# roljon/Steered-Mixture-of-Experts

Hardware: AMD Instinct MI355X
Metric: Mpixel-iters/s (SMoE fit: forward + analytic backward + TF1 Adam), 16x16 blocks / 4 kernels (higher is better)
Workload: dtype f32

## Files before the change

### steered_mixture_of_experts_amd/csrc/smoe_block.hip.h

```cpp
#ifndef SMOE_BLOCK_HIP_H
#define SMOE_BLOCK_HIP_H

#include <hip/hip_runtime.h>
#include <stdint.h>

#include <type_traits>

#include "smoe_device.h"
#include "smoe_ssim.hip.h"
#include "smoe_fq.hip.h"

namespace smoe {


__device__ __forceinline__ float fast_rcp(float x) { return __builtin_amdgcn_rcpf(x); }

__device__ __forceinline__ uint32_t hw_wave_slot() {
    return __builtin_amdgcn_s_getreg(4 | (0 << 6) | ((4 - 1) << 11));
}
__device__ __forceinline__ void rotate_priority(int it, uint32_t slot) {
    const uint32_t pr = ((uint32_t)it + slot) % 3u;
    if (pr == 0u) __builtin_amdgcn_s_setprio(0);
    else if (pr == 1u) __builtin_amdgcn_s_setprio(1);
    else __builtin_amdgcn_s_setprio(2);
// ... 51 lines not shown
        case 2: return s.A_diagonal;
        case 3: return s.A_corr;
        case 4: return s.gamma_e;
        default: return s.nu_e;
    }
}

#ifndef SMOE_REGRED
#define SMOE_REGRED 0
#endif
#ifndef SMOE_W2_SLOTS
#define SMOE_W2_SLOTS 96
#endif
#ifndef SMOE_W2_G16
#define SMOE_W2_G16 1
#endif
#ifndef SMOE_W2_G32
#define SMOE_W2_G32 1
#endif
#ifndef SMOE_W2_SLOTS_MAX
#define SMOE_W2_SLOTS_MAX 150
#endif
#ifndef SMOE_NT_STORES
#define SMOE_NT_STORES 1
#endif
#ifndef SMOE_SGPR_CONSTS
#define SMOE_SGPR_CONSTS 1
#endif
#ifndef SMOE_PHASE_CLOCKS
#define SMOE_PHASE_CLOCKS 0
#endif
#if SMOE_PHASE_CLOCKS
#define SMOE_CLK(i) do { const unsigned long long _t = __builtin_amdgcn_s_memtime(); clk[i] += (float)(_t - clk_last); clk_last = __builtin_amdgcn_s_memtime(); } while (0)
#else
#define SMOE_CLK(i) do { } while (0)
#endif
#ifndef SMOE_DEBUG
#define SMOE_DEBUG 0
#endif
#if SMOE_DEBUG
#define SMOE_LDS_CHECK(end_floats, code)                                                   \
    do {                                                                                   \
        if ((long)(end_floats) > (long)a.lds_floats) {                                     \
            if (threadIdx.x == 0 && a.dbg != nullptr) atomicOr(a.dbg, (uint32_t)(code));   \
            return;                                                                        \
        }                                                                                  \
    } while (0)
#else
#define SMOE_LDS_CHECK(end_floats, code) do { } while (0)
#endif
#define SMOE_SQ 0.84932180028801904272f
#define SMOE_INV_SQ 1.17740022503374817543f

template <int D, int C, int K>
struct BlockRegs {
    using Lt = Layout<D, C, K>;
    float P[Lt::LP_STRIDE];
    float As[K][Lt::TRI];
    float cz[K][D];
    float coef[K];
    float hz[K][D];
    float he[K][C];
    float hq[K];

    __device__ __forceinline__ float pi(int k) const { return P[k * Lt::PK + Lt::O_PI]; }
    __device__ __forceinline__ float mu(int k, int l) const { return P[k * Lt::PK + Lt::O_MU + l]; }
    __device__ __forceinline__ float A(int k, int l, int m) const { return P[k * Lt::PK + Lt::O_A + tri_index(l, m)]; }
    __device__ __forceinline__ float nu(int k, int c) const { return P[k * Lt::PK + Lt::O_NU + c]; }
    __device__ __forceinline__ float ga(int k, int l, int c) const { return P[k * Lt::PK + Lt::O_GA + l * C + c]; }
    __device__ __forceinline__ bool flag(int k) const { return P[Lt::LP_ACT + k] != 0.0f; }
    __device__ __forceinline__ bool frozen() const { return P[Lt::LP_FROZEN] != 0.0f; }
    __device__ __forceinline__ bool act(int k) const { return flag(k) && (pi(k) > 0.0f); }

    __device__ __forceinline__ void load(const float* __restrict__ lds_block) {
        const float4* src = reinterpret_cast<const float4*>(lds_block);
#pragma unroll
        for (int i = 0; i < Lt::LP_STRIDE / 4; ++i) {
            const float4 q = src[i];
            P[4 * i + 0] = q.x; P[4 * i + 1] = q.y; P[4 * i + 2] = q.z; P[4 * i + 3] = q.w;
        }
    }

    template <bool IC = false>
    __device__ __forceinline__ void derive(const KernelConsts& kc) {
#pragma unroll
        for (int k = 0; k < K; ++k) {
            float det = 1.0f;
#pragma unroll
            for (int l = 0; l < D; ++l) det *= A(k, l, l);
            const float nq = kc.use_det ? det * kc.inv_n_dis : 1.0f;
            coef[k] = act(k) ? nq * pi(k) : 0.0f;
#pragma unroll
            for (int l = 0; l < D; ++l)
#pragma unroll
                for (int m = 0; m <= l; ++m)
                    As[k][tri_index(l, m)] = (IC ? ((l == m) ? SMOE_SQ * SMOE_SQ : 2.0f * SMOE_SQ * SMOE_SQ) : SMOE_SQ) * A(k, l, m);
#pragma unroll
            for (int m = 0; m < D; ++m) {
                float c = 0.0f;
                if (!IC) {
#pragma unroll
                    for (int l = m; l < D; ++l) c = fmaf(mu(k, l), As[k][tri_index(l, m)], c);
                }
                cz[k][m] = c;
            }
            if (!kc.train_gammas) {
#pragma unroll
                for (int i = 0; i < D * C; ++i) P[k * Lt::PK + Lt::O_GA + i] = 0.0f;
            }
            if (kc.only_y_gamma) {
#pragma unroll
                for (int l = 0; l < D; ++l)
#pragma unroll
                    for (int c = 1; c < C; ++c) P[k * Lt::PK + Lt::O_GA + l * C + c] = 0.0f;
            }
        }
    }
};

template <int D, int C, int K>
struct BlockRanges {
    FqRange ad, ac, mu, nu, ga;
    float lo[5], hi[5];
    __device__ __forceinline__ void compute(const float* P, const bool (&keep)[K], const KernelConsts& kc) {
        using Lt = Layout<D, C, K>;
        constexpr float INF = __builtin_huge_valf();
#pragma unroll
        for (int t = 0; t < 5; ++t) { lo[t] = INF; hi[t] = -INF; }
        bool any = false;
#pragma unroll
        for (int k = 0; k < K; ++k) {
            if (!keep[k]) continue;
            any = true;
            const float* p = P + k * Lt::PK;
#pragma unroll
            for (int l = 0; l < D; ++l) {
                lo[2] = fminf(lo[2], p[Lt::O_MU + l]); hi[2] = fmaxf(hi[2], p[Lt::O_MU + l]);
#pragma unroll
                for (int m = 0; m <= l; ++m) {
                    const float a = p[Lt::O_A + tri_index(l, m)];
                    const int t = (l == m) ? 0 : 1;
                    lo[t] = fminf(lo[t], a); hi[t] = fmaxf(hi[t], a);
                }
            }
#pragma unroll
            for (int c = 0; c < C; ++c) { lo[3] = fminf(lo[3], p[Lt::O_NU + c]); hi[3] = fmaxf(hi[3], p[Lt::O_NU + c]); }
#pragma unroll
            for (int i = 0; i < D * C; ++i) { lo[4] = fminf(lo[4], p[Lt::O_GA + i]); hi[4] = fmaxf(hi[4], p[Lt::O_GA + i]); }
        }
// ... 241 lines not shown
#pragma unroll
            for (int l = m; l < D - HL; ++l)
                a[Lt::O_A + tri_index(l, m)] = fmaf(x[l], uz, a[Lt::O_A + tri_index(l, m)]);
        }
        }
#pragma unroll
        for (int c = 0; c < C; ++c) {
            a[Lt::O_NU + c] = fmaf(o.wt[k], Gc[c], a[Lt::O_NU + c]);
#pragma unroll
            for (int l = 0; l < D - HL; ++l)
                a[Lt::O_GA + l * C + c] = fmaf(o.wt[k], Gx[l][c], a[Lt::O_GA + l * C + c]);
        }
    }
}

template <int D, int C, int K, int HL, bool IC = false>
__device__ __forceinline__ void complete_const(const BlockRegs<D, C, K>& R, const float (&xc)[D], float* __restrict__ acc) {
    using Lt = Layout<D, C, K>;
#pragma unroll
    for (int k = 0; k < K; ++k) {
        float* a = acc + k * Lt::PK;
        if (!IC) {
#pragma unroll
            for (int m = D - HL; m < D; ++m) a[Lt::O_MU + m] = R.hz[k][m] * a[Lt::O_PI];
        }
#pragma unroll
        for (int l = D - HL; l < D; ++l) {
            if (IC) {
                const float rl = xc[l] - R.mu(k, l);
#pragma unroll
                for (int m = 0; m <= l; ++m)
                    a[Lt::O_A + tri_index(l, m)] = (m < D - HL) ? rl * a[Lt::O_MU + m] : rl * ((xc[m] - R.mu(k, m)) * a[Lt::O_PI]);
                a[Lt::O_MU + l] = rl * a[Lt::O_PI];
            } else {
#pragma unroll
            for (int m = 0; m <= l; ++m) a[Lt::O_A + tri_index(l, m)] = xc[l] * a[Lt::O_MU + m];
            }
#pragma unroll
            for (int c = 0; c < C; ++c) a[Lt::O_GA + l * C + c] = xc[l] * a[Lt::O_NU + c];
        }
    }
}

template <int D, int C, int K>
__device__ __forceinline__ void tie_diagonal(float* __restrict__ a) {
    using Lt = Layout<D, C, K>;
    float tr = 0.0f;
#pragma unroll
    for (int l = 0; l < D; ++l) tr += a[Lt::O_A + tri_index(l, l)];
#pragma unroll
    for (int l = 0; l < D; ++l) a[Lt::O_A + tri_index(l, l)] = tr;
}

template <int D, int C, int K, bool IC = false>
__device__ __forceinline__ void finish_partials(const BlockRegs<D, C, K>& R, const KernelConsts& kc,
                                                float* __restrict__ acc) {
    using Lt = Layout<D, C, K>;
#pragma unroll
    for (int k = 0; k < K; ++k) {
        float* a = acc + k * Lt::PK;
        const bool act = R.act(k);
        const float su = a[Lt::O_PI];
        if (IC) {
            float sur[D];
#pragma unroll
            for (int l = 0; l < D; ++l) sur[l] = a[Lt::O_MU + l];
#pragma unroll
            for (int l = 0; l < D; ++l) {
                float gm = 0.0f;
#pragma unroll
                for (int m = 0; m < D; ++m) gm = fmaf((l >= m) ? R.A(k, l, m) : R.A(k, m, l), sur[m], gm);
                a[Lt::O_MU + l] = gm;
#pragma unroll
                for (int m = 0; m <= l; ++m) {
                    float v = (l == m) ? -0.5f * a[Lt::O_A + tri_index(l, m)] : -a[Lt::O_A + tri_index(l, m)];
                    if (l == m && kc.use_det) v = fmaf(su, act ? fast_rcp(R.A(k, l, l)) : 0.0f, v);
                    a[Lt::O_A + tri_index(l, m)] = v;
                }
            }
            a[Lt::O_PI] = su * (act ? fast_rcp(R.pi(k)) : 0.0f);
            if (kc.radial) tie_diagonal<D, C, K>(a);
            continue;
        }
        float suz[D];
#pragma unroll
        for (int m = 0; m < D; ++m) suz[m] = a[Lt::O_MU + m] * SMOE_INV_SQ;
#pragma unroll
        for (int l = 0; l < D; ++l) {
            float gm = 0.0f;
#pragma unroll
            for (int m = 0; m <= l; ++m) gm = fmaf(R.A(k, l, m), suz[m], gm);
            a[Lt::O_MU + l] = gm;
        }
#pragma unroll
        for (int l = 0; l < D; ++l) {
#pragma unroll
            for (int m = 0; m <= l; ++m) {
                float v = fmaf(R.mu(k, l), suz[m], -(a[Lt::O_A + tri_index(l, m)] * SMOE_INV_SQ));
                if (l == m && kc.use_det) v = fmaf(su, act ? fast_rcp(R.A(k, l, l)) : 0.0f, v);
                a[Lt::O_A + tri_index(l, m)] = v;
            }
        }
        a[Lt::O_PI] = su * (act ? fast_rcp(R.pi(k)) : 0.0f);
        if (kc.radial) tie_diagonal<D, C, K>(a);
    }
}

struct SlotDesc {
    float c_self, pub_scale;
    uint32_t T1, T2, T3, TR, P1, P2, P3, PR, FLAG, PIV;
};

template <int D, int C, int K, bool IC>
__device__ __forceinline__ SlotDesc build_slot_desc(int j, uint32_t tot_base, uint32_t img_base, uint32_t par_base,
                                                    bool patch_pis, bool use_det) {
    using Lt = Layout<D, C, K>;
    const uint32_t ZERO = par_base + 4u * Lt::LP_ZERO, ONE = par_base + 4u * Lt::LP_ONE;
    const int k = j / Lt::PK, o = j - k * Lt::PK;
    const uint32_t Tk = tot_base + 4u * (uint32_t)(k * Lt::PK), Pk = img_base + 4u * (uint32_t)(k * Lt::PK);
    SlotDesc d;
    d.c_self = 1.0f; d.pub_scale = 1.0f;
    d.T1 = d.T2 = d.T3 = d.TR = ZERO;
    d.P1 = d.P2 = d.P3 = ZERO;
    d.PR = ONE;
    d.FLAG = img_base + 4u * (uint32_t)(Lt::LP_ACT + k);
    d.PIV = patch_pis ? par_base + 4u * (uint32_t)(Lt::LP_QPI + k) : Pk + 4u * Lt::O_PI;
    if (o == Lt::O_PI) {
        d.c_self = 0.0f; d.TR = Tk + 4u * Lt::O_PI; d.PR = d.PIV;
    } else if (o < Lt::O_A) {
        const int l = o - Lt::O_MU;
        d.c_self = 0.0f;
        d.pub_scale = IC ? 1.0f : SMOE_INV_SQ;
        int n = 0;
#pragma unroll
        for (int m = 0; m < D; ++m) {
            if (IC || m <= l) {
                const int hi = (l > m) ? l : m, lo = (l > m) ? m : l;
                const uint32_t P = Pk + 4u * (uint32_t)(Lt::O_A + hi * (hi + 1) / 2 + lo), T = Tk + 4u * (uint32_t)(Lt::O_MU + m);
                if (n == 0) { d.P1 = P; d.T1 = T; } else if (n == 1) { d.P2 = P; d.T2 = T; } else { d.P3 = P; d.T3 = T; }
                ++n;
            }
        }
    } else if (o < Lt::O_NU) {
        const int t = o - Lt::O_A;
        const int l = (t >= 3) ? 2 : ((t >= 1) ? 1 : 0);
        const int m = t - l * (l + 1) / 2;
        if (IC) {
            d.c_self = (l == m) ? -0.5f : -1.0f;
        } else {
            d.c_self = -SMOE_INV_SQ;
            d.P1 = Pk + 4u * (uint32_t)(Lt::O_MU + l);
            d.T1 = Tk + 4u * (uint32_t)(Lt::O_MU + m);
        }
        if (l == m && use_det) { d.TR = Tk + 4u * Lt::O_PI; d.PR = Pk + 4u * (uint32_t)(Lt::O_A + l * (l + 1) / 2 + l); }
    }
    return d;
// ... 21 lines not shown
        return (t == 0) ? 1 : ((t == 1) ? D : ((t == 2 || t == 3) ? D * D : ((t == 4) ? D * C : C)));
    }
    __host__ __device__ static constexpr int before(int t) {
        int n = 0;
        for (int u = 0; u < t; ++u) n += elems(u);
        return n;
    }
    static constexpr int PER_KERNEL = before(6);
};

template <int D, int C, int K, int G, int WAVES>
struct Tile {
    using Lt = Layout<D, C, K>;
    static constexpr int BPW = 64 / G;
    static constexpr int NB = WAVES * BPW;
    static constexpr int U = (G == 64) ? ((Lt::NSLOT >= 90) ? 16 : 32) : G;
    static constexpr int UL = G / U;
    static constexpr int RPR = 64 / UL / (64 / G);
    static constexpr int NROUND = (Lt::NSLOT + RPR - 1) / RPR;
    static constexpr int CH = RPR;
    static constexpr int RPP = CH / RPR;
    static constexpr int ROW = 64 + 4;
    static constexpr int NCHUNK = (Lt::NSLOT + CH - 1) / CH;
    static constexpr bool REGRED = (G == 64) && (SMOE_REGRED != 0);
    static constexpr int RM = (Lt::NSLOT + 3) / 4;
    static constexpr int SPL = REGRED ? (RM + 15) / 16 : (NROUND + UL - 1) / UL;
    __host__ __device__ static constexpr int slot_of(int sub, int s) {
        if (REGRED) {
            const int i = (sub % 16) + 16 * s;
            return (i < RM) ? (sub / 16) * RM + i : Lt::NSLOT;
        }
        return (UL * s + (sub % UL)) * RPR + sub / UL;
    }
    static constexpr int THREADS = WAVES * 64;
    static constexpr int FWD_PXR = 16;
    static_assert(NB * K * ParamTile<D, C, K>::PER_KERNEL <= WAVES * CH * ROW, "the parameter tile of a workgroup is staged in the reduction scratch");
    static constexpr int MV_STRIDE = round_up(2 * Lt::NPAR, 4);
    static constexpr int TGT_PAD = 0;
    __host__ __device__ static constexpr int tgt_stride(int N) { return C * N + TGT_PAD; }
    __host__ __device__ static constexpr int lw_stride(int N) { return N + TGT_PAD; }
    
    __host__ __device__ static int off_coords() { return 0; }
    __host__ __device__ static int off_par(int N, int CR) { return round_up(CR * N, 4); }
    __host__ __device__ static int off_mv(int N, int CR) { return off_par(N, CR) + NB * Lt::LP_STRIDE; }
    static constexpr bool OWNER_POST = (G >= 64);
    static constexpr int DESC_DW = 12;
    static constexpr int DESC_STRIDE = OWNER_POST ? Lt::NPAR * DESC_DW : 0;
    static constexpr int TOT_STRIDE = round_up(Lt::NSLOT, 4);
    static_assert(!OWNER_POST || BPW * TOT_STRIDE <= CH * ROW, "the published totals must fit into the reduction scratch");
    __host__ __device__ static bool wants_owner_post(int N) { return OWNER_POST && N <= 8 * G; }
    __host__ __device__ static int off_scratch(int N, int CR) { return off_mv(N, CR) + NB * MV_STRIDE; }
    __host__ __device__ static int off_tgt(int N, int CR) { return off_scratch(N, CR) + WAVES * CH * ROW; }
    __host__ __device__ static int off_lw(int N, int CR) { return off_tgt(N, CR) + NB * tgt_stride(N); }
    __host__ __device__ static size_t bytes(int N, bool has_lw, int CR = D, bool hq = false) {
        return sizeof(float) * (size_t)off_ssim(N, has_lw, CR, hq);
    }
    static constexpr int QI_RNG = 40;
    static constexpr int QI_OUT = 12;
    static constexpr int QI_STRIDE = round_up(Lt::LP_STRIDE + QI_RNG + QI_OUT, 4);
    __host__ __device__ static int off_qimg(int N, bool has_lw, int CR) { return round_up(off_lw(N, CR) + (has_lw ? NB * lw_stride(N) : 0), 4); }
    __host__ __device__ static int off_ssim(int N, bool has_lw, int CR, bool hq = false) { return off_qimg(N, has_lw, CR) + (hq ? NB * QI_STRIDE : 0); }
    __host__ __device__ static int ssim_tabs(int bh, int bw, int bt = 0) { return (G == 16) ? 0 : round_up(11 * (bh + bw + bt), 4); }
    __host__ __device__ static int ssim_wave(int N) { return (G == 16) ? BPW * C * N : round_up(C * N + ((D == 3) ? 10 : 8) * N, 4); }
    __host__ __device__ static size_t bytes_ssim(int N, bool has_lw, int CR, int bh, int bw, bool hq = false, int bt = 0) {
        return sizeof(float) * (size_t)(off_ssim(N, has_lw, CR, hq) + ssim_tabs(bh, bw, bt) + WAVES * ssim_wave(N));
    }
};

template <int D, int C, int K, int G, int WAVES, int CR = D>
__device__ __forceinline__ void stage_inputs(const float* __restrict__ coords, const float* __restrict__ target,
                                             const float* __restrict__ loss_w, int B, int N, int blk0,
                                             float* __restrict__ lds, bool planes = true) {
    using T = Tile<D, C, K, G, WAVES>;
    static_assert(T::TGT_PAD == 0, "the staged planes of a workgroup are one contiguous run");
    float* s_coords = lds + T::off_coords();
    float* s_tgt = lds + T::off_tgt(N, CR);
    float* s_lw = lds + T::off_lw(N, CR);
    auto copy_planes = [&](const float* __restrict__ src, float* __restrict__ dst, int per) {
        const size_t g0 = (size_t)blk0 * per;
        const size_t gend = (size_t)B * per;
        if ((per & 3) == 0) {
            const float4* __restrict__ src4 = reinterpret_cast<const float4*>(src);
            const size_t last4 = (gend >> 2) - 1;
            for (int i = threadIdx.x; i < T::NB * (per >> 2); i += T::THREADS)
                reinterpret_cast<float4*>(dst)[i] = src4[min((g0 >> 2) + (size_t)i, last4)];
        } else {
            for (int i = threadIdx.x; i < T::NB * per; i += T::THREADS) dst[i] = src[min(g0 + (size_t)i, gend - 1)];
        }
    };
    for (int i = threadIdx.x; i < CR * N; i += T::THREADS) s_coords[i] = coords[i];
    if (!planes) return;
    copy_planes(target, s_tgt, C * N);
    if (loss_w != nullptr) copy_planes(loss_w, s_lw, N);
}

template <int D, int C, int K, int NB, int THREADS>
struct TileIO {
    using PT = ParamTile<D, C, K>;
    static constexpr int TOTAL = NB * K * PT::PER_KERNEL;
    static constexpr int MAXE = (TOTAL + THREADS - 1) / THREADS;
    __device__ static __forceinline__ void locate(int i, int& t, int& local) {
        t = 0; local = i;
#pragma unroll
        for (int u = 1; u < 6; ++u)
            if (i >= NB * K * PT::before(u)) { t = u; local = i - NB * K * PT::before(u); }
    }
    __device__ static __forceinline__ void fetch(const smoe_params& s, int blk0, int B, float (&v)[MAXE]) {
#pragma unroll
        for (int e = 0; e < MAXE; ++e) {
// ... 340 lines not shown
            for (int l = 0; l < D; ++l) x[l] = (l < D - HL) ? s_coords[l * N + n] : 0.0f;
#pragma unroll
            for (int c = 0; c < C; ++c) t[c] = s_tgt[c * N + n];
            const float lw = HAS_LW ? s_lw[n] : 1.0f;
            PixelOut<D, C, K> o;
            pixel<D, C, K, true, HL, false, IC, false, RAWL>(R, kc, x, t, lw, acc, o, nullptr, nullptr, !(HAS_LW && sample) || lw != 0.0f, lraw);
        }
    }
    if constexpr (RAWL) {
#pragma unroll
        for (int c = 0; c < C; ++c) acc[Layout<D, C, K>::S_LOSS] = fmaf(kc.cw[c], lraw[c], acc[Layout<D, C, K>::S_LOSS]);
    }
    const int lane = threadIdx.x & 63;
#pragma unroll
    for (int k = 0; k < K; ++k) acc[Layout<D, C, K>::S_CNT + k] += ((flags[k] >> lane) & 1ull) ? 1.0f : 0.0f;
}

template <int D, int C, int K, int G, int HL, bool SSIM, bool QUANT>
constexpr int fit_min_waves() {
    return ((G == 64 || (G == 16 && SMOE_W2_G16) || (G == 32 && SMOE_W2_G32)) && HL >= 1 && !SSIM && !QUANT && Layout<D, C, K>::NSLOT >= ((G == 64) ? SMOE_W2_SLOTS : 90)
            && Layout<D, C, K>::NSLOT <= SMOE_W2_SLOTS_MAX) ? 2 : 1;
}

template <int D, int C, int K, int G, int WAVES, int HL, bool SSIM = false, bool QUANT = false, bool IC = false, bool PAIR = false>
__global__ void __launch_bounds__(WAVES * 64) __attribute__((amdgpu_waves_per_eu(fit_min_waves<D, C, K, G, HL, SSIM, QUANT>()))) fit_kernel(FitArgs a) {
    using Lt = Layout<D, C, K>;
    using T = Tile<D, C, K, G, WAVES>;
    static_assert(!PAIR || (G == 64 && WAVES == 2 && !SSIM && !QUANT), "PAIR: one block on the two wavefronts of a workgroup");
    extern __shared__ __attribute__((aligned(16))) float lds[];
    const int N = a.N;
    const int B = a.B;
    const int wave = threadIdx.x >> 6;
    const int lane = threadIdx.x & 63;
    const int grp = lane / G;
    const int sub = lane - grp * G;
    const int blk0 = blockIdx.x * (PAIR ? 1 : T::NB);
    const int lb = PAIR ? 0 : wave * T::BPW + grp;
    const bool helper = PAIR && wave != 0;
    const int b_raw = blk0 + lb;
    const bool valid_b = b_raw < B;
    const int b = valid_b ? b_raw : B - 1;

    constexpr int CR = D - HL;
    float* s_coords = lds + T::off_coords();
    float* s_par = lds + T::off_par(N, CR) + lb * Lt::LP_STRIDE;
    float* s_mv = lds + T::off_mv(N, CR) + lb * T::MV_STRIDE;
    float* s_scratch = lds + T::off_scratch(N, CR) + wave * (T::CH * T::ROW);
    const bool owner_post = T::OWNER_POST && a.desc_off > 0;
    float* s_desc = lds + a.desc_off + lb * T::DESC_STRIDE;
    float* s_tot = s_scratch + grp * T::TOT_STRIDE;
    const float* s_tgt = lds + T::off_tgt(N, CR) + lb * T::tgt_stride(N);
    const float* s_lw = lds + T::off_lw(N, CR) + lb * T::lw_stride(N);
    const bool has_lw = a.loss_w != nullptr;

    SMOE_LDS_CHECK(T::off_ssim(N, has_lw, CR, QUANT) + (SSIM ? T::ssim_tabs(a.bh, a.bw, (D == 3) ? a.bt : 0) + WAVES * T::ssim_wave(N) : 0), 1u);
    if (owner_post) SMOE_LDS_CHECK(a.desc_off + T::NB * T::DESC_STRIDE, 2u);
    stage_inputs<D, C, K, G, WAVES, CR>(a.coords, a.target, a.loss_w, B, N, blk0, lds);
    float* s_q = lds + T::off_qimg(N, has_lw, CR) + lb * T::QI_STRIDE;
    float* s_rng = s_q + Lt::LP_STRIDE;
    float* s_out = s_rng + T::QI_RNG;
    float* s_ssim = lds + T::off_ssim(N, has_lw, CR, QUANT);
    const int bh = a.bh, bw = a.bw, bt = (D == 3) ? a.bt : 0;
    const float* s_Tr = s_ssim;
    const float* s_Tc = s_ssim + bh * 11;
    const float* s_Tt = s_Tc + bw * 11;
    float* s_X = s_ssim + T::ssim_tabs(bh, bw, bt) + wave * T::ssim_wave(N) + ((G == 16) ? grp * (C * N) : 0);
    float* s_Wa = s_X + C * N;
    float* s_Wb = s_Wa + 5 * N;
    float wj[11];
    if (SSIM) {
        if (G == 16) {
#pragma unroll
            for (int q = 0; q < 11; ++q) {
                wj[q] = a.ssim_T[11 * 16 + sub * 11 + q];
            }
        } else {
            for (int i = threadIdx.x; i < 11 * (bh + bw + bt); i += T::THREADS) s_ssim[i] = a.ssim_T[i];
        }
    }
    float xc[D];
#pragma unroll
    for (int l = 0; l < D; ++l) xc[l] = a.coords[l * N + min(sub, N - 1)];

    constexpr int QS = QUANT ? T::SPL : 1;
    float lr[T::SPL], reg[T::SPL], qlo[QS], qhi[QS], qsc[QS], qiv[QS];
    float goff[QS];
    int meta[T::SPL], qt[QS];
#pragma unroll
    for (int s = 0; s < QS; ++s) {
        qlo[s] = -__builtin_huge_valf(); qhi[s] = __builtin_huge_valf();
        qsc[s] = qiv[s] = 0.0f;
        qt[s] = -1;
        goff[s] = 0.0f;
    }
#pragma unroll
    for (int s = 0; s < T::SPL; ++s) {
        const int j = T::slot_of(sub, s);
        lr[s] = reg[s] = 0.0f;
        meta[s] = -1;
        if (j < Lt::NPAR) {
            int tensor, kern; long off;
            decode_slot<D, C, K>(j, b, tensor, off, kern);
            s_par[j] = pick(a.p, tensor)[off];
            s_mv[2 * j] = pick(a.m, tensor)[off];
            s_mv[2 * j + 1] = pick(a.v, tensor)[off];
            float r = (tensor == 0) ? a.lr_pis : ((tensor == 2 || tensor == 3) ? a.lr_steer : a.lr_expert);
            if (tensor == 0 && !a.train_pis) r = 0.0f;
            if (tensor == 1 && !a.train_musx) r = 0.0f;
// ... 66 lines not shown
                        o[0] = r.nmin; o[1] = r.nmax; o[2] = r.scale; o[3] = r.inv;
                        o[4] = r.back; o[5] = r.zero ? 1.0f : 0.0f; o[6] = lo; o[7] = hi;
                    }
                }
                wave_lds_sync();
            }
        }
        if constexpr (!QUANT) {
#pragma unroll
            for (int s = 0; s < T::SPL; ++s) {
                const int j = T::slot_of(sub, s);
                if (meta[s] >= 0 && (meta[s] & 15) == 0) {
                    const float x = s_par[j];
                    const float cl = fminf(fmaxf(x, a.kc.q_nmin[3]), a.kc.q_nmax[3]);
                    s_par[Lt::LP_QPI + (meta[s] >> 4)] = floorf((cl - a.kc.q_nmin[3]) * a.kc.q_inv[3] + 0.5f) * a.kc.q_scale[3] + a.kc.q_nmin[3];
                }
            }
            wave_lds_sync();
            return;
        }
        if constexpr (QUANT) {
#pragma unroll
        for (int s = 0; s < T::SPL; ++s) {
            const int j = T::slot_of(sub, s);
            if (j < Lt::NPAR) {
                const float x = s_par[j] - goff[s];
                float q = x;
                if (qsc[s] != 0.0f) {
                    const float cl = fminf(fmaxf(x, qlo[s]), qhi[s]);
                    q = floorf((cl - qlo[s]) * qiv[s] + 0.5f) * qsc[s] + qlo[s];
                }
                {
                    if (qt[s] >= 0) {
                        const float* o = s_rng + qt[s] * 8;
                        FqRange r;
                        r.nmin = o[0]; r.nmax = o[1]; r.scale = o[2]; r.inv = o[3]; r.back = o[4]; r.zero = o[5] != 0.0f;
                        r.shift = (qt[s] == 0 && a.kc.radial) ? 0.0f : r.back;
                        q = fq_val(x, r);
                    }
                }
                s_q[j] = q + goff[s];
            } else if (j >= Lt::S_CNT && j < Lt::S_CNT + K) {
                s_q[Lt::LP_ACT + (j - Lt::S_CNT)] = s_par[Lt::LP_ACT + (j - Lt::S_CNT)];
            } else if (j == Lt::S_LOSS) {
                s_q[Lt::LP_FROZEN] = s_par[Lt::LP_FROZEN];
            }
        }
        }
        wave_lds_sync();
    };
    if (has_quant) refresh_quantised_image();
    const float* s_img = (QUANT && has_quant) ? s_q : s_par;
    const bool patch_pis = !QUANT && (a.kc.qpis != 0);
    if (owner_post && !helper) {
        const uint32_t tot_off = (uint32_t)((s_tot - lds) * sizeof(float));
        const uint32_t img_off = (uint32_t)((s_img - lds) * sizeof(float));
        const uint32_t par_off = (uint32_t)((s_par - lds) * sizeof(float));
#pragma unroll
        for (int s = 0; s < T::SPL; ++s) {
            const int j = T::slot_of(sub, s);
            if (j < Lt::NPAR) {
                const SlotDesc d = build_slot_desc<D, C, K, IC>(j, tot_off, img_off, par_off, patch_pis, a.kc.use_det != 0);
                float4* o = reinterpret_cast<float4*>(s_desc + j * T::DESC_DW);
                o[0] = make_float4(d.c_self, d.pub_scale, __uint_as_float(d.T1), __uint_as_float(d.T2));
                o[1] = make_float4(__uint_as_float(d.T3), __uint_as_float(d.TR), __uint_as_float(d.P1), __uint_as_float(d.P2));
                o[2] = make_float4(__uint_as_float(d.P3), __uint_as_float(d.PR), __uint_as_float(d.FLAG), __uint_as_float(d.PIV));
            } else if (j == Lt::S_LOSS) {
                s_par[Lt::LP_ZERO] = 0.0f;
                s_par[Lt::LP_ONE] = 1.0f;
            }
        }
        wave_lds_sync();
    }

    float b1p = a.b1p, b2p = a.b2p;
    const KernelConsts kc = a.kc;
    const float beta1 = a.beta1, beta2 = a.beta2, adam_eps = a.eps, clip = a.clip;
    const float reg_pi = a.reg_pi, reg_u = a.reg_u;

#if SMOE_PHASE_CLOCKS
    float clk[8] = {0.0f, 0.0f, 0.0f, 0.0f, 0.0f, 0.0f, 0.0f, 0.0f};
    unsigned long long clk_last = __builtin_amdgcn_s_memtime();
#endif
    const bool phase_prio = !PAIR && (G < 64 || N >= 8 * G);
    for (int it = 0; it < a.n_iters; ++it) {
        if (a.prio_rotate) rotate_priority(it, hw_wave_slot());
        else if (phase_prio) __builtin_amdgcn_s_setprio(0);
        float acc[Lt::NSLOT];
#pragma unroll
        for (int j = 0; j < Lt::NSLOT; ++j) acc[j] = 0.0f;
        bool frozen;
        float reg_loss = 0.0f;
        {
            BlockRegs<D, C, K> R;
            R.load(s_img);
            if (patch_pis) {
#pragma unroll
                for (int k = 0; k < K; ++k) R.P[k * Lt::PK + Lt::O_PI] = R.P[Lt::LP_QPI + k];
            }
            R.template derive<IC>(kc);
            frozen = R.frozen();
            if (has_reg) {
                const float rp = kc.kcount_norm ? kc.pis_l1_raw / count_pis<D, C, K>(R.P) : reg_pi;
#pragma unroll
                for (int k = 0; k < K; ++k) {
                    if (R.act(k)) {
                        reg_loss += rp * R.pi(k);
#pragma unroll
                        for (int l = 0; l < D; ++l) reg_loss += reg_u * R.A(k, l, l);
                    }
                }
            }
            if (HL > 0) hoist_const<D, C, K, HL, IC>(R, xc);
#if SMOE_SGPR_CONSTS
            if constexpr (G == 64 && !SSIM && !QUANT && !IC && HL >= 1 && K * C >= 24) {
                auto uni = [](float x) { return __int_as_float(__builtin_amdgcn_readfirstlane(__float_as_int(x))); };
#pragma unroll
                for (int k = 0; k < K; ++k) {
                    R.coef[k] = uni(R.coef[k]);
#pragma unroll
                    for (int l = 0; l < D - HL; ++l) {
#pragma unroll
                        for (int m = 0; m <= l; ++m) R.As[k][tri_index(l, m)] = uni(R.As[k][tri_index(l, m)]);
#pragma unroll
                        for (int c = 0; c < C; ++c) R.P[k * Lt::PK + Lt::O_GA + l * C + c] = uni(R.P[k * Lt::PK + Lt::O_GA + l * C + c]);
                    }
                }
            }
#endif
            SMOE_CLK(0);
            if constexpr (SSIM) {
                const int pxl = (N + G - 1) / G;
                const int full = (G == 16) ? N / G : 0;
                auto recon_step = [&](int n) {
                    float x[D], t[C], scratch_acc[Lt::NSLOT];
#pragma unroll
                    for (int l = 0; l < D; ++l) x[l] = (l < D - HL) ? s_coords[l * N + n] : 0.0f;
#pragma unroll
                    for (int c = 0; c < C; ++c) t[c] = s_tgt[c * N + n];
#pragma unroll
                    for (int j = 0; j < Lt::NSLOT; ++j) scratch_acc[j] = 0.0f;
                    PixelOut<D, C, K> o;
                    pixel<D, C, K, false, HL, false, IC>(R, kc, x, t, 1.0f, scratch_acc, o);
#pragma unroll
                    for (int c = 0; c < C; ++c) s_X[c * N + n] = o.q[c];
                };
                for (int i = 0; i < full; ++i) recon_step(i * G + sub);
                for (int i = full; i < pxl; ++i)
                    if (i * G + sub < N) recon_step(i * G + sub);
                wave_lds_sync();
                if constexpr (G == 16) acc[Lt::S_LOSS] = ssim_block16<C, true>(s_X, s_tgt, sub, wj, kc.sw);
                else if constexpr (D == 3) acc[Lt::S_LOSS] = ssim_block3<C, true>(s_X, s_tgt, s_Wa, s_Wb, s_Tr, s_Tc, s_Tt, kc.sw, bh, bw, bt, N, lane);
                else acc[Lt::S_LOSS] = ssim_block<C, true>(s_X, s_tgt, s_Wa, s_Wb, s_Tr, s_Tc, kc.sw, bh, bw, N, lane);
                unsigned long long flags[K];
#pragma unroll
                for (int k = 0; k < K; ++k) flags[k] = 0ull;
                auto grad_step = [&](int n, auto voted) {
                    float x[D], t[C], gq[C];
#pragma unroll
                    for (int l = 0; l < D; ++l) x[l] = (l < D - HL) ? s_coords[l * N + n] : 0.0f;
#pragma unroll
                    for (int c = 0; c < C; ++c) { t[c] = s_tgt[c * N + n]; gq[c] = s_X[c * N + n]; }
                    PixelOut<D, C, K> o;
                    pixel<D, C, K, true, HL, true, IC, decltype(voted)::value>(R, kc, x, t, 1.0f, acc, o, gq, flags);
                };
                for (int i = 0; i < full; ++i) grad_step(i * G + sub, std::true_type{});
                for (int i = full; i < pxl; ++i)
                    if (i * G + sub < N) grad_step(i * G + sub, std::false_type{});
#pragma unroll
                for (int k = 0; k < K; ++k) acc[Lt::S_CNT + k] += ((flags[k] >> lane) & 1ull) ? 1.0f : 0.0f;
            } else {
                const int gl = PAIR ? 2 * G : G, sl = PAIR ? wave * G + sub : sub;
                if (has_lw) pixel_loop_train<D, C, K, true, HL, IC>(R, kc, s_coords, s_tgt, s_lw, N, gl, sl, acc, a.lw_is_sample != 0);
                else pixel_loop_train<D, C, K, false, HL, IC>(R, kc, s_coords, s_tgt, s_lw, N, gl, sl, acc);
            }
            if (HL > 0) complete_const<D, C, K, HL, IC>(R, xc, acc);
            SMOE_CLK(1);
        }
        if (phase_prio) __builtin_amdgcn_s_setprio(3);
        if (!owner_post) {
            BlockRegs<D, C, K> R2;
            R2.load(s_img);
            if (patch_pis) {
#pragma unroll
                for (int k = 0; k < K; ++k) R2.P[k * Lt::PK + Lt::O_PI] = R2.P[Lt::LP_QPI + k];
            }
            finish_partials<D, C, K, IC>(R2, kc, acc);
        }

        SMOE_CLK(2);
        float total[T::SPL];
        reduce_slots<D, C, K, G, WAVES, 0>(acc, s_scratch, lane, total);
        SMOE_CLK(3);

        if constexpr (PAIR) {
            float* s_x = lds + T::off_scratch(N, CR) + (T::CH * T::ROW);
            if (helper) {
                wave_lds_sync();
#pragma unroll
                for (int s = 0; s < T::SPL; ++s) {
                    const int j = T::slot_of(sub, s);
                    if (j < Lt::NSLOT) s_x[j] = total[s];
                }
            }
            __syncthreads();
            if (helper) {
                __syncthreads();
                b1p *= beta1;
                b2p *= beta2;
                SMOE_CLK(4);
                continue;
            }
#pragma unroll
            for (int s = 0; s < T::SPL; ++s) {
                const int j = T::slot_of(sub, s);
                if (j < Lt::NSLOT) total[s] += s_x[j];
            }
        }

        SMOE_CLK(4);
        if (owner_post) {
            SlotDesc dsc[T::SPL];
#pragma unroll
            for (int s = 0; s < T::SPL; ++s) {
                int j = T::slot_of(sub, s);
                asm volatile("" : "+v"(j));
                const int jc = (j < Lt::NPAR) ? j : 0;
                const float4* q = reinterpret_cast<const float4*>(s_desc + jc * T::DESC_DW);
                const float4 q0 = q[0], q1 = q[1], q2 = q[2];
                dsc[s].c_self = q0.x; dsc[s].pub_scale = q0.y; dsc[s].T1 = __float_as_uint(q0.z); dsc[s].T2 = __float_as_uint(q0.w);
                dsc[s].T3 = __float_as_uint(q1.x); dsc[s].TR = __float_as_uint(q1.y); dsc[s].P1 = __float_as_uint(q1.z); dsc[s].P2 = __float_as_uint(q1.w);
                dsc[s].P3 = __float_as_uint(q2.x); dsc[s].PR = __float_as_uint(q2.y); dsc[s].FLAG = __float_as_uint(q2.z); dsc[s].PIV = __float_as_uint(q2.w);
                if (j < Lt::NPAR) s_tot[j] = total[s] * dsc[s].pub_scale;
            }
            wave_lds_sync();
#pragma unroll
            for (int s = 0; s < T::SPL; ++s) {
                const int j = T::slot_of(sub, s);
                if (j < Lt::NPAR) total[s] = eval_slot_desc(lds, dsc[s], total[s]);
            }
// ... 87 lines not shown
                        float g = (bel[s] || abv[s]) ? 0.0f : gq[s];
                        g += tlo[s] ? pick5(rs, 0, qt[s]) / fmaxf(pick5(cn, 0, qt[s]), 1.0f) : 0.0f;
                        g += thi[s] ? pick5(rs, 5, qt[s]) / fmaxf(pick5(cn, 5, qt[s]), 1.0f) : 0.0f;
                        gq[s] = g;
                    }
                }
            }
        }
        float newp[T::SPL], newm[T::SPL], newv[T::SPL], pvs[T::SPL], mvs[T::SPL], vvs[T::SPL];
#pragma unroll
        for (int s = 0; s < T::SPL; ++s) {
            const int j = T::slot_of(sub, s);
            const int jc = (j < Lt::NPAR) ? j : 0;
            pvs[s] = s_par[jc];
            mvs[s] = s_mv[2 * jc];
            vvs[s] = s_mv[2 * jc + 1];
        }
        bool bad = false;
#pragma unroll
        for (int s = 0; s < T::SPL; ++s) {
            const int j = T::slot_of(sub, s);
            const float pv = pvs[s], mv = mvs[s], vv = vvs[s];
            float gsum = gq[s];
            if constexpr (QUANT) {
                gsum = (pv - goff[s] >= qlo[s] && pv - goff[s] <= qhi[s]) ? gsum : 0.0f;
            } else {
                if (patch_pis && meta[s] >= 0 && (meta[s] & 15) == 0) gsum = (pv >= kc.q_nmin[3] && pv <= kc.q_nmax[3]) ? gsum : 0.0f;
            }
            if (clip > 0.0f) gsum = fminf(fmaxf(gsum, -clip), clip);
            const float alpha = lr[s] * bias;
            const float m2 = mv + (gsum - mv) * (1.0f - beta1);
            const float v2 = vv + (gsum * gsum - vv) * (1.0f - beta2);
            const float p2 = pv - (m2 * alpha) * fast_rcp(__builtin_amdgcn_sqrtf(v2) + adam_eps);
            const bool upd = (j < Lt::NPAR) && (lr[s] != 0.0f) && !frozen;
            newp[s] = upd ? p2 : pv;
            newm[s] = upd ? m2 : mv;
            newv[s] = upd ? v2 : vv;
            const float lossv = (SSIM ? 1.0f + total[s] : total[s]) + reg_loss;
            const bool is_loss = (j == Lt::S_LOSS) && !frozen;
            last_loss = is_loss ? lossv : last_loss;
            bad = bad || (is_loss && ((lossv != lossv) || (has_loss0 && (lossv + 1.0f > (loss0 + 100.0f) * 10.0f))));
            last_sse = ((j == Lt::S_SSE) && !frozen) ? total[s] : last_sse;
        }
        wave_lds_sync();
        SMOE_CLK(6);
#pragma unroll
        for (int s = 0; s < T::SPL; ++s) {
            const int j = T::slot_of(sub, s);
            if (j < Lt::NPAR) {
                s_par[j] = newp[s];
                s_mv[2 * j] = newm[s];
                s_mv[2 * j + 1] = newv[s];
                if constexpr (!QUANT) {
                    if (patch_pis && meta[s] >= 0 && (meta[s] & 15) == 0) {
                        const float cl = fminf(fmaxf(newp[s], kc.q_nmin[3]), kc.q_nmax[3]);
                        s_par[Lt::LP_QPI + (meta[s] >> 4)] = floorf((cl - kc.q_nmin[3]) * kc.q_inv[3] + 0.5f) * kc.q_scale[3] + kc.q_nmin[3];
                    }
                }
            } else if (j >= Lt::S_CNT && j < Lt::S_CNT + K) {
                if (!frozen) s_par[Lt::LP_ACT + (j - Lt::S_CNT)] = (total[s] > 0.0f) ? 1.0f : 0.0f;
            } else if (j == Lt::S_LOSS) {
                if (bad) s_par[Lt::LP_FROZEN] = 1.0f;
            }
        }
        wave_lds_sync();
        if constexpr (QUANT) {
            if (has_quant) refresh_quantised_image();
        }
        if constexpr (PAIR) __syncthreads();
        b1p *= beta1;
        b2p *= beta2;
        SMOE_CLK(7);
    }
#if SMOE_PHASE_CLOCKS
    if (blockIdx.x == 0 && lane == 0 && a.loss_out != nullptr) {
#pragma unroll
        for (int i = 0; i < 8; ++i) a.loss_out[B / 2 + wave * 8 + i] = clk[i];
    }
    return;
#endif

    const FitArgs* ka = (const FitArgs*)__builtin_amdgcn_kernarg_segment_ptr();
    asm volatile("" : "+s"(ka));
    if (valid_b && !helper) {
        int bo = b;
        asm volatile("" : "+v"(bo));
#pragma unroll
        for (int s = 0; s < T::SPL; ++s) {
            const int j = T::slot_of(sub, s);
            if (j < Lt::NPAR) {
                int tensor, kern; long off;
                decode_slot<D, C, K>(j, bo, tensor, off, kern);
                pick(ka->p, tensor)[off] = s_par[j];
                pick(ka->m, tensor)[off] = s_mv[2 * j];
                pick(ka->v, tensor)[off] = s_mv[2 * j + 1];
            } else if (j == Lt::S_LOSS) {
                if (ka->loss_out != nullptr && made_a_pass(last_loss)) ka->loss_out[b] = last_loss;
                if (ka->diverged != nullptr) ka->diverged[b] = (s_par[Lt::LP_FROZEN] != 0.0f) ? 1u : 0u;
                uint32_t mask = 0u;
#pragma unroll
                for (int k = 0; k < K; ++k) mask |= (s_par[Lt::LP_ACT + k] != 0.0f) ? (1u << k) : 0u;
                ka->active[b] = mask;
            } else if (j == Lt::S_SSE) {
                if (ka->sse_out != nullptr && made_a_pass(last_sse)) ka->sse_out[b] = last_sse;
            }
        }
    }
}

typedef float smoe_f4 __attribute__((ext_vector_type(4)));
// ... 370 lines not shown
}

template <typename Args>
hipError_t launch_with_lds(void (*kern)(Args), int grid, int threads, size_t lds, Args a, hipStream_t st) {
    const hipError_t e = allow_lds(reinterpret_cast<const void*>(kern), lds);
    if (e != hipSuccess) return e;
    a.lds_floats = (int)(lds / sizeof(float));
    hipLaunchKernelGGL(kern, dim3(grid), dim3(threads), lds, st, a);
    return hipGetLastError();
}

template <typename Args>
int resident_workgroups(void (*kern)(Args), int threads, size_t lds) {
    int nb = 0;
    if (allow_lds(reinterpret_cast<const void*>(kern), lds) != hipSuccess) return -1;
    if (hipOccupancyMaxActiveBlocksPerMultiprocessor(&nb, kern, threads, lds) != hipSuccess) return -1;
    return nb;
}

template <typename Args>
struct Launch {
    void (*kern)(Args) = nullptr;
    int hl = 0;
    int threads = 0, nb = 1;
    size_t lds = 0;
    int desc_off = 0;
    int regt = 0;
};

template <int D, int C, int K, int G, int WAVES, bool SSIM, bool QUANT, bool IC, bool PAIR, int HMIN, int HMAX>
auto fit_kernel_at(int hl) -> void (*)(FitArgs) {
    if constexpr (HMAX > HMIN) {
        if (hl < HMAX) return fit_kernel_at<D, C, K, G, WAVES, SSIM, QUANT, IC, PAIR, HMIN, HMAX - 1>(hl);
    }
    return fit_kernel<D, C, K, G, WAVES, HMAX, SSIM, QUANT, IC, PAIR>;
}

template <int D, int C, int K, int G, int WAVES, bool SSIM, bool QUANT, bool IC, int OM, int HMAX>
auto forward_kernel_at(int hl) -> void (*)(FwdArgs) {
    if constexpr (HMAX > 0) {
        if (hl < HMAX) return forward_kernel_at<D, C, K, G, WAVES, SSIM, QUANT, IC, OM, HMAX - 1>(hl);
    }
    return forward_kernel<D, C, K, G, WAVES, SSIM, QUANT, IC, HMAX, OM>;
}

template <int D, int C, int K, int G, int WAVES, bool FULL>
Launch<FitArgs> resolve_fit(Graph g, int N, bool has_lw, int hoist, int bh, int bw, int bt) {
    using T = Tile<D, C, K, G, WAVES>;
    constexpr int HMAX = (D == 3) ? 2 : 1;
    Launch<FitArgs> r;
    r.threads = T::THREADS;
    r.nb = T::NB;
    size_t shm = 0;
    if (g.ssim) {
        if constexpr (FULL && (D == 2 || (D == 3 && G == 64))) {
            if (G == 16 && (bh != 16 || bw != 16 || hoist < 1)) return r;
            constexpr int H0 = (G == 16) ? 1 : 0;
            r.hl = (hoist >= 1) ? 1 : H0;
            r.kern = g.quant ? (g.ic ? fit_kernel_at<D, C, K, G, WAVES, true, true, true, false, H0, 1>(r.hl)
                                     : fit_kernel_at<D, C, K, G, WAVES, true, true, false, false, H0, 1>(r.hl))
                             : (g.ic ? fit_kernel_at<D, C, K, G, WAVES, true, false, true, false, H0, 1>(r.hl)
                                     : fit_kernel_at<D, C, K, G, WAVES, true, false, false, false, H0, 1>(r.hl));
            shm = T::bytes_ssim(N, has_lw, D - r.hl, bh, bw, g.quant, (D == 3) ? bt : 0);
        } else {
            return r;
        }
    } else {
        r.hl = (hoist >= HMAX) ? HMAX : ((hoist >= 1) ? 1 : 0);
        if (g.quant) {
            if constexpr (FULL) {
                r.kern = g.ic ? fit_kernel_at<D, C, K, G, WAVES, false, true, true, false, 0, HMAX>(r.hl)
                              : fit_kernel_at<D, C, K, G, WAVES, false, true, false, false, 0, HMAX>(r.hl);
            } else {
                return r;
            }
        } else if (g.ic) {
            r.kern = fit_kernel_at<D, C, K, G, WAVES, false, false, true, false, 0, HMAX>(r.hl);
        } else {
            r.kern = fit_kernel_at<D, C, K, G, WAVES, false, false, false, false, 0, HMAX>(r.hl);
            if constexpr (G == 64 && WAVES == 2) {
                if (g.pair) {
                    r.kern = fit_kernel_at<D, C, K, G, WAVES, false, false, false, true, 0, HMAX>(r.hl);
                    r.nb = 1;
                }
            }
        }
        shm = T::bytes(N, has_lw, D - r.hl, g.quant);
    }
    if (T::wants_owner_post(N)) {
        r.desc_off = (int)(shm / sizeof(float));
        shm += sizeof(float) * (size_t)T::NB * T::DESC_STRIDE;
    }
    r.lds = shm;
    return r;
}

template <int D, int C, int K, int G, int WAVES, bool FULL>
Launch<FwdArgs> resolve_fwd(Graph g, int N, bool has_lw, int hoist, int bh, int bw, int bt) {
    using T = Tile<D, C, K, G, WAVES>;
    constexpr int HMAX = (D == 3) ? 2 : 1;
    Launch<FwdArgs> r;
    r.threads = T::THREADS;
    r.nb = T::NB;
    if (g.ssim) {
        if constexpr (FULL && (D == 2 || (D == 3 && G == 64))) {
            if (G == 16 && (bh != 16 || bw != 16)) return r;
            r.kern = g.quant ? (g.ic ? forward_kernel<D, C, K, G, WAVES, true, true, true> : forward_kernel<D, C, K, G, WAVES, true, true>)
                             : (g.ic ? forward_kernel<D, C, K, G, WAVES, true, false, true> : forward_kernel<D, C, K, G, WAVES, true>);
            r.lds = T::bytes_ssim(N, has_lw, D, bh, bw, false, (D == 3) ? bt : 0);
        }
        return r;
    }
    r.hl = (hoist >= HMAX) ? HMAX : ((hoist >= 1) ? 1 : 0);
    if (g.quant) {
        if constexpr (FULL) {
            if (r.hl > 1) r.hl = 1;
            r.kern = g.ic ? forward_kernel_at<D, C, K, G, WAVES, false, true, true, 0, 1>(r.hl)
                          : forward_kernel_at<D, C, K, G, WAVES, false, true, false, 0, 1>(r.hl);
        } else {
            return r;
        }
    } else if (g.ic) {
        r.kern = forward_kernel_at<D, C, K, G, WAVES, false, false, true, 0, HMAX>(r.hl);
    } else {
        r.kern = g.outs ? forward_kernel_at<D, C, K, G, WAVES, false, false, false, 2, HMAX>(r.hl)
                        : forward_kernel_at<D, C, K, G, WAVES, false, false, false, 1, HMAX>(r.hl);
    }
    r.regt = ((N + G - 1) / G <= T::FWD_PXR) ? 1 : 0;
    r.lds = r.regt ? sizeof(float) * (size_t)T::off_tgt(N, D - r.hl) : T::bytes(N, has_lw, D - r.hl);
    return r;
}

template <int D, int C, int K, int G, int WAVES, bool FULL>
hipError_t launch_fit(const FitArgs& a, Graph g, int hoist, hipStream_t st) {
    const Launch<FitArgs> r = resolve_fit<D, C, K, G, WAVES, FULL>(g, a.N, a.loss_w != nullptr, hoist, a.bh, a.bw, a.bt);
    if (!r.kern) return hipErrorNotSupported;
    FitArgs aa = a;
    aa.desc_off = r.desc_off;
    return launch_with_lds(r.kern, (a.B + r.nb - 1) / r.nb, r.threads, r.lds, aa, st);
}

template <int D, int C, int K, int G, int WAVES, bool FULL>
hipError_t launch_fwd(const FwdArgs& a, Graph g, hipStream_t st) {
    const Launch<FwdArgs> r = resolve_fwd<D, C, K, G, WAVES, FULL>(g, a.N, a.loss_w != nullptr, a.hoist, a.bh, a.bw, a.bt);
    if (!r.kern) return hipErrorNotSupported;
    FwdArgs aa = a;
    aa.regt = r.regt;
    return launch_with_lds(r.kern, (a.B + r.nb - 1) / r.nb, r.threads, r.lds, aa, st);
}

template <int D, int C, int K, int G, int WAVES, bool FULL>
size_t lds_bytes(Graph g, int N, bool has_lw, int bh, int bw, int bt) {
    if (!g.ssim) return Tile<D, C, K, G, WAVES>::bytes(N, has_lw, D, g.quant);
    if (!FULL || !(D == 2 || (D == 3 && G == 64)) || (G == 16 && (bh != 16 || bw != 16))) return (size_t)-1;
    return Tile<D, C, K, G, WAVES>::bytes_ssim(N, has_lw, D, bh, bw, g.quant, (D == 3) ? bt : 0);
}

template <int D, int C, int K, int G, int WAVES, bool FULL>
int fit_occupancy(int N, bool has_lw, int hoist, bool pair) {
    Graph g = {};
    g.pair = pair;
    const Launch<FitArgs> r = resolve_fit<D, C, K, G, WAVES, FULL>(g, N, has_lw, hoist, 0, 0, 0);
    const int nb = resident_workgroups(r.kern, r.threads, r.lds);
    return (nb < 0) ? -1 : nb * WAVES;
}

#define SMOE_STR_(x) #x
#define SMOE_STR(x) SMOE_STR_(x)
#define SMOE_VARIANT(D, C, K, G, W, FULL) \
    { D, C, K, G, W, "fit_d" SMOE_STR(D) "c" SMOE_STR(C) "k" SMOE_STR(K) "_g" SMOE_STR(G) "w" SMOE_STR(W), (FULL) != 0, \
      &launch_fit<D, C, K, G, W, (FULL) != 0>, &launch_fwd<D, C, K, G, W, (FULL) != 0>, &lds_bytes<D, C, K, G, W, (FULL) != 0>, \
      &fit_occupancy<D, C, K, G, W, (FULL) != 0>, &launch_readmit_quant<D, C, K, G, W>, \
      team_fit_ptr<D, C, K, G, W>(), team_lds_ptr<D, C, K, G, W>(), team_occ_ptr<D, C, K, G, W>(), \
      duo_fit_ptr<D, C, K, G>(), duo_lds_ptr<D, C, K, G>(), duo_occ_ptr<D, C, K, G>(), \
      &launch_render<D, C, K, (SMOE_FULL != 0)>, &launch_render_blend<D, C, K, (SMOE_FULL != 0)> }

}
#endif
```

Measured before the change: 410,200.

## Cache derived Cholesky constants and reciprocals in an LDS image per block

Adds a per-block LDS 'derived image' that holds the scaled A entries and the reciprocals of the diagonal A entries and pi. Owner lanes publish these values whenever parameters are updated in the Adam step. Every pixel lane then loads them with float4 reads instead of recomputing the scaling and rcp in derive and finish_partials. This cuts redundant per-lane ALU work but costs extra LDS space, which may lower occupancy, plus additional stores and a wave sync.

```diff
diff --git a/steered_mixture_of_experts_amd/csrc/smoe_block.hip.h b/steered_mixture_of_experts_amd/csrc/smoe_block.hip.h
--- a/steered_mixture_of_experts_amd/csrc/smoe_block.hip.h
+++ b/steered_mixture_of_experts_amd/csrc/smoe_block.hip.h
@@ -127,6 +127,22 @@
 #define SMOE_SQ 0.84932180028801904272f
 #define SMOE_INV_SQ 1.17740022503374817543f
 
+#ifndef SMOE_DERIVED
+#define SMOE_DERIVED 1
+#endif
+template <int D, int C, int K, int G>
+constexpr int derived_level() {
+    return (SMOE_DERIVED != 0 && (C == 1 || G == 64) && !(G == 64 && K * C >= 24)) ? 1 : 0;
+}
+template <int D, int C, int K>
+struct DerivedImage {
+    using Lt = Layout<D, C, K>;
+    static constexpr int O_AS = 0;
+    static constexpr int O_RCP = round_up(K * Lt::TRI, 4);
+    static constexpr int STRIDE = O_RCP + round_up(K * (D + 1), 4);
+    static constexpr int N_AS = O_RCP, N_RCP = STRIDE - O_RCP;
+};
+
 template <int D, int C, int K>
 struct BlockRegs {
     using Lt = Layout<D, C, K>;
@@ -156,8 +172,9 @@
         }
     }
 
-    template <bool IC = false>
-    __device__ __forceinline__ void derive(const KernelConsts& kc) {
+    template <bool IC = false, int DER = 0>
+    __device__ __forceinline__ void derive(const KernelConsts& kc, const float* __restrict__ das = nullptr) {
+        static_assert(!(IC && DER != 0), "the derived image holds the constants of the plain graph");
 #pragma unroll
         for (int k = 0; k < K; ++k) {
             float det = 1.0f;
@@ -168,8 +185,11 @@
 #pragma unroll
             for (int l = 0; l < D; ++l)
 #pragma unroll
-                for (int m = 0; m <= l; ++m)
+                for (int m = 0; m <= l; ++m) {
+                    if constexpr (DER != 0) As[k][tri_index(l, m)] = das[DerivedImage<D, C, K>::O_AS + k * Lt::TRI + tri_index(l, m)];
+                    else
                     As[k][tri_index(l, m)] = (IC ? ((l == m) ? SMOE_SQ * SMOE_SQ : 2.0f * SMOE_SQ * SMOE_SQ) : SMOE_SQ) * A(k, l, m);
+                }
 #pragma unroll
             for (int m = 0; m < D; ++m) {
                 float c = 0.0f;
@@ -517,10 +537,11 @@
     for (int l = 0; l < D; ++l) a[Lt::O_A + tri_index(l, l)] = tr;
 }
 
-template <int D, int C, int K, bool IC = false>
+template <int D, int C, int K, bool IC = false, int DER = 0>
 __device__ __forceinline__ void finish_partials(const BlockRegs<D, C, K>& R, const KernelConsts& kc,
-                                                float* __restrict__ acc) {
+                                                float* __restrict__ acc, const float* __restrict__ drc = nullptr) {
     using Lt = Layout<D, C, K>;
+    static_assert(!(IC && DER != 0), "the derived image holds the constants of the plain graph");
 #pragma unroll
     for (int k = 0; k < K; ++k) {
         float* a = acc + k * Lt::PK;
@@ -562,11 +583,17 @@
 #pragma unroll
             for (int m = 0; m <= l; ++m) {
                 float v = fmaf(R.mu(k, l), suz[m], -(a[Lt::O_A + tri_index(l, m)] * SMOE_INV_SQ));
-                if (l == m && kc.use_det) v = fmaf(su, act ? fast_rcp(R.A(k, l, l)) : 0.0f, v);
+                if (l == m && kc.use_det) {
+                    float ra;
+                    if constexpr (DER != 0) ra = drc[k * (D + 1) + 1 + l]; else ra = fast_rcp(R.A(k, l, l));
+                    v = fmaf(su, act ? ra : 0.0f, v);
+                }
                 a[Lt::O_A + tri_index(l, m)] = v;
             }
         }
-        a[Lt::O_PI] = su * (act ? fast_rcp(R.pi(k)) : 0.0f);
+        float rp;
+        if constexpr (DER != 0) rp = drc[k * (D + 1)]; else rp = fast_rcp(R.pi(k));
+        a[Lt::O_PI] = su * (act ? rp : 0.0f);
         if (kc.radial) tie_diagonal<D, C, K>(a);
     }
 }
@@ -694,9 +721,12 @@
     __host__ __device__ static int off_scratch(int N, int CR) { return off_mv(N, CR) + NB * MV_STRIDE; }
     __host__ __device__ static int off_tgt(int N, int CR) { return off_scratch(N, CR) + WAVES * CH * ROW; }
     __host__ __device__ static int off_lw(int N, int CR) { return off_tgt(N, CR) + NB * tgt_stride(N); }
-    __host__ __device__ static size_t bytes(int N, bool has_lw, int CR = D, bool hq = false) {
-        return sizeof(float) * (size_t)off_ssim(N, has_lw, CR, hq);
-    }
+    __host__ __device__ static size_t bytes(int N, bool has_lw, int CR = D, bool hq = false, bool der = false) {
+        return sizeof(float) * (size_t)(off_ssim(N, has_lw, CR, hq) + (der ? NB * DER_STRIDE : 0));
+    }
+    static constexpr int DER = derived_level<D, C, K, G>();
+    static constexpr int DER_STRIDE = DER ? DerivedImage<D, C, K>::STRIDE : 0;
+    __host__ __device__ static int off_der(int N, bool has_lw, int CR) { return off_qimg(N, has_lw, CR); }
     static constexpr int QI_RNG = 40;
     static constexpr int QI_OUT = 12;
     static constexpr int QI_STRIDE = round_up(Lt::LP_STRIDE + QI_RNG + QI_OUT, 4);
@@ -1143,8 +1173,12 @@
     const float* s_tgt = lds + T::off_tgt(N, CR) + lb * T::tgt_stride(N);
     const float* s_lw = lds + T::off_lw(N, CR) + lb * T::lw_stride(N);
     const bool has_lw = a.loss_w != nullptr;
-
-    SMOE_LDS_CHECK(T::off_ssim(N, has_lw, CR, QUANT) + (SSIM ? T::ssim_tabs(a.bh, a.bw, (D == 3) ? a.bt : 0) + WAVES * T::ssim_wave(N) : 0), 1u);
+    constexpr int DER = (!SSIM && !QUANT && !IC && !PAIR) ? T::DER : 0;
+    using DI = DerivedImage<D, C, K>;
+    float* s_der = lds + T::off_der(N, has_lw, CR) + lb * T::DER_STRIDE;
+
+    SMOE_LDS_CHECK(T::off_ssim(N, has_lw, CR, QUANT) + (DER ? T::NB * T::DER_STRIDE : 0)
+                   + (SSIM ? T::ssim_tabs(a.bh, a.bw, (D == 3) ? a.bt : 0) + WAVES * T::ssim_wave(N) : 0), 1u);
     if (owner_post) SMOE_LDS_CHECK(a.desc_off + T::NB * T::DESC_STRIDE, 2u);
     stage_inputs<D, C, K, G, WAVES, CR>(a.coords, a.target, a.loss_w, B, N, blk0, lds);
     float* s_q = lds + T::off_qimg(N, has_lw, CR) + lb * T::QI_STRIDE;
@@ -1317,6 +1351,28 @@
     if (has_quant) refresh_quantised_image();
     const float* s_img = (QUANT && has_quant) ? s_q : s_par;
     const bool patch_pis = !QUANT && (a.kc.qpis != 0);
+    auto publish_own = [&](int s, float v, float piv) {
+        if constexpr (DER != 0) {
+            if (meta[s] < 0) return;
+            const int tensor = meta[s] & 15, k = meta[s] >> 4;
+            if (tensor == 2 || tensor == 3) {
+                const int t = T::slot_of(sub, s) - k * Lt::PK - Lt::O_A;
+                s_der[DI::O_AS + k * Lt::TRI + t] = SMOE_SQ * v;
+                const int l = (t >= 3) ? 2 : ((t >= 1) ? 1 : 0);
+                if (tensor == 2) s_der[DI::O_RCP + k * (D + 1) + 1 + l] = fast_rcp(v);
+            } else if (tensor == 0) {
+                s_der[DI::O_RCP + k * (D + 1)] = fast_rcp(piv);
+            }
+        }
+    };
+    if constexpr (DER != 0) {
+#pragma unroll
+        for (int s = 0; s < T::SPL; ++s) {
+            const int j = T::slot_of(sub, s);
+            if (j < Lt::NPAR) publish_own(s, s_par[j], patch_pis ? s_par[Lt::LP_QPI + (meta[s] >> 4)] : s_par[j]);
+        }
+        wave_lds_sync();
+    }
     if (owner_post && !helper) {
         const uint32_t tot_off = (uint32_t)((s_tot - lds) * sizeof(float));
         const uint32_t img_off = (uint32_t)((s_img - lds) * sizeof(float));
@@ -1363,7 +1419,18 @@
 #pragma unroll
                 for (int k = 0; k < K; ++k) R.P[k * Lt::PK + Lt::O_PI] = R.P[Lt::LP_QPI + k];
             }
-            R.template derive<IC>(kc);
+            if constexpr (DER != 0) {
+                float das[DI::N_AS];
+                const float4* src = reinterpret_cast<const float4*>(s_der + DI::O_AS);
+#pragma unroll
+                for (int i = 0; i < DI::N_AS / 4; ++i) {
+                    const float4 q = src[i];
+                    das[4 * i + 0] = q.x; das[4 * i + 1] = q.y; das[4 * i + 2] = q.z; das[4 * i + 3] = q.w;
+                }
+                R.template derive<IC, DER>(kc, das);
+            } else {
+                R.template derive<IC>(kc);
+            }
             frozen = R.frozen();
             if (has_reg) {
                 const float rp = kc.kcount_norm ? kc.pis_l1_raw / count_pis<D, C, K>(R.P) : reg_pi;
@@ -1450,7 +1517,18 @@
 #pragma unroll
                 for (int k = 0; k < K; ++k) R2.P[k * Lt::PK + Lt::O_PI] = R2.P[Lt::LP_QPI + k];
             }
-            finish_partials<D, C, K, IC>(R2, kc, acc);
+            if constexpr (DER != 0) {
+                float drc[DI::N_RCP];
+                const float4* src = reinterpret_cast<const float4*>(s_der + DI::O_RCP);
+#pragma unroll
+                for (int i = 0; i < DI::N_RCP / 4; ++i) {
+                    const float4 q = src[i];
+                    drc[4 * i + 0] = q.x; drc[4 * i + 1] = q.y; drc[4 * i + 2] = q.z; drc[4 * i + 3] = q.w;
+                }
+                finish_partials<D, C, K, IC, DER>(R2, kc, acc, drc);
+            } else {
+                finish_partials<D, C, K, IC>(R2, kc, acc);
+            }
         }
 
         SMOE_CLK(2);
@@ -1644,10 +1722,13 @@
                 s_mv[2 * j] = newm[s];
                 s_mv[2 * j + 1] = newv[s];
                 if constexpr (!QUANT) {
+                    float piv = newp[s];
                     if (patch_pis && meta[s] >= 0 && (meta[s] & 15) == 0) {
                         const float cl = fminf(fmaxf(newp[s], kc.q_nmin[3]), kc.q_nmax[3]);
-                        s_par[Lt::LP_QPI + (meta[s] >> 4)] = floorf((cl - kc.q_nmin[3]) * kc.q_inv[3] + 0.5f) * kc.q_scale[3] + kc.q_nmin[3];
+                        piv = floorf((cl - kc.q_nmin[3]) * kc.q_inv[3] + 0.5f) * kc.q_scale[3] + kc.q_nmin[3];
+                        s_par[Lt::LP_QPI + (meta[s] >> 4)] = piv;
                     }
+                    publish_own(s, newp[s], piv);
                 }
             } else if (j >= Lt::S_CNT && j < Lt::S_CNT + K) {
                 if (!frozen) s_par[Lt::LP_ACT + (j - Lt::S_CNT)] = (total[s] > 0.0f) ? 1.0f : 0.0f;
@@ -2124,6 +2205,7 @@
     r.threads = T::THREADS;
     r.nb = T::NB;
     size_t shm = 0;
+    bool der = false;
     if (g.ssim) {
         if constexpr (FULL && (D == 2 || (D == 3 && G == 64))) {
             if (G == 16 && (bh != 16 || bw != 16 || hoist < 1)) return r;
@@ -2150,14 +2232,16 @@
             r.kern = fit_kernel_at<D, C, K, G, WAVES, false, false, true, false, 0, HMAX>(r.hl);
         } else {
             r.kern = fit_kernel_at<D, C, K, G, WAVES, false, false, false, false, 0, HMAX>(r.hl);
+            der = true;
             if constexpr (G == 64 && WAVES == 2) {
                 if (g.pair) {
                     r.kern = fit_kernel_at<D, C, K, G, WAVES, false, false, false, true, 0, HMAX>(r.hl);
                     r.nb = 1;
-                }
-            }
-        }
-        shm = T::bytes(N, has_lw, D - r.hl, g.quant);
+                    der = false;
+                }
+            }
+        }
+        shm = T::bytes(N, has_lw, D - r.hl, g.quant, der);
     }
     if (T::wants_owner_post(N)) {
         r.desc_off = (int)(shm / sizeof(float));
@@ -2223,7 +2307,7 @@
 
 template <int D, int C, int K, int G, int WAVES, bool FULL>
 size_t lds_bytes(Graph g, int N, bool has_lw, int bh, int bw, int bt) {
-    if (!g.ssim) return Tile<D, C, K, G, WAVES>::bytes(N, has_lw, D, g.quant);
+    if (!g.ssim) return Tile<D, C, K, G, WAVES>::bytes(N, has_lw, D, g.quant, !g.quant && !g.ic);
     if (!FULL || !(D == 2 || (D == 3 && G == 64)) || (G == 16 && (bh != 16 || bw != 16))) return (size_t)-1;
     return Tile<D, C, K, G, WAVES>::bytes_ssim(N, has_lw, D, bh, bw, g.quant, (D == 3) ? bt : 0);
 }
```

Result: no change. 408,400 (-0.4%).
